# kit-cel/vae-equalizer

Hardware: AMD Instinct MI355X
Metric: equalized symbols/s/GPU, DP 64-QAM VAE-LE (higher is better)
Workload: dtype f32

## Files before the change

### vae_equalizer_amd/csrc/vaeq_dp_wave_kernel.h

```cpp
#pragma once
#include <hip/hip_runtime.h>
#include <stdint.h>
#include <type_traits>

#include "vaeq.h"
#include "vaeq_common.h"
#include "vaeq_launch.h"
#include "vaeq_wave.h"

#ifdef VAEQ_PHASE_STAMPS
#define VAEQ_STAMP(i) do { if (s == a.steps - 1) tst[i] = __builtin_readcyclecounter(); } while (0)
#define VAEQ_XSTAMP(i) do { if (s == a.steps - 1) tsx[i] = __builtin_readcyclecounter(); } while (0)
#else
#define VAEQ_STAMP(i) do { } while (0)
#define VAEQ_XSTAMP(i) do { } while (0)
#endif
#define VAEQ_NSTAMP 12
#ifndef VAEQ_PIPE
#define VAEQ_PIPE 1
#endif
#ifndef VAEQ_PIPE_DU
#define VAEQ_PIPE_DU 0
#endif
#ifndef VAEQ_ROW_STEP
#define VAEQ_ROW_STEP 1
#endif
#define VAEQ_BT_FRAMES 16
#ifndef VAEQ_DEMAP_SHIFT
#define VAEQ_DEMAP_SHIFT 0
#endif
#ifndef VAEQ_WPS
#define VAEQ_WPS 2
#endif
#ifndef VAEQ_CHAIN_BOUND
#define VAEQ_CHAIN_BOUND 0
#endif
#ifndef VAEQ_HALF_SWAP
#define VAEQ_HALF_SWAP 1
#endif
#ifndef VAEQ_QST_OFF
#define VAEQ_QST_OFF 0
#endif
#ifndef VAEQ_QST_NOWAIT
#define VAEQ_QST_NOWAIT 1
#endif
#ifndef VAEQ_QST_NT
#define VAEQ_QST_NT 1
#endif

namespace vaeq {

#if VAEQ_CHAIN_BOUND
__device__ __forceinline__ float chain_sum(float v) { asm volatile("" :: "v"(v)); return 1.0f; }
__device__ __forceinline__ float chain_scan(float v) { return v; }
__device__ __forceinline__ float chain_half_scan(float v) { return v; }
__device__ __forceinline__ float chain_rcp(float v) { asm volatile("" :: "v"(v)); return 1.0f; }
__device__ __forceinline__ float chain_log(float v) { asm volatile("" :: "v"(v)); return 1.0f; }
__device__ __forceinline__ void chain_adam(float &, float &m, float &v, float g, float, float) { m = g; v = g; }
#define VAEQ_CUT(real, cut) (cut)
#else
#define VAEQ_CUT(real, cut) (real)
__device__ __forceinline__ float chain_sum(float v) { return wave_sum_dpp(v); }
__device__ __forceinline__ float chain_scan(float v) { return wave_incl_scan_dpp(v); }
__device__ __forceinline__ float chain_half_scan(float v) { return half_incl_scan_dpp(v); }
__device__ __forceinline__ float chain_rcp(float v) { return __builtin_amdgcn_rcpf(v); }
__device__ __forceinline__ float chain_log(float v) { return __builtin_amdgcn_logf(v); }
__device__ __forceinline__ void chain_adam(float &p, float &m, float &v, float g, float ss, float bc) { adam_update_fast(p, m, v, g, ss, bc); }
#endif

template <bool DH>
__device__ __forceinline__ float half_sum(float a0, float a1, int half)
{
#if VAEQ_CHAIN_BOUND
    if constexpr (DH) return half ? a1 : a0;
#endif
    const auto r = __builtin_amdgcn_permlane32_swap(__builtin_bit_cast(unsigned, a0), __builtin_bit_cast(unsigned, a1), false, false);
    return __builtin_bit_cast(float, (unsigned)r[0]) + __builtin_bit_cast(float, (unsigned)r[1]);
}

struct WaveLayout {
    int Lph, Uph;
    int X, E, U, PSv, W, H, PSh, VS, MOM, RED, XG, total;
};

__host__ __device__ inline WaveLayout wave_layout(int B, int M, int NW = 1)
{
    WaveLayout l;
    const int len = 2 * B + M - 1;
    const int lph = wave_lph(len);
    l.Lph = lph;
    l.Uph = B / 2 + 1;
    int o = 0;
    auto take = [&](int bytes) { int r = o; o += (bytes + 15) & ~15; return r; };
    l.X = take(2 * 4 * lph * 8);
    l.E = take(2 * 4 * lph * 8);
    const int ubytes = 2 * 2 * l.Uph * 8, gbytes = 2 * B * 8;
    l.U = take(ubytes > gbytes ? ubytes : gbytes);
    l.PSv = take(2 * (B + 1) * 4);
    l.W = take(2 * M * 16);
    l.H = take(2 * 2 * (M + 1) * 8);
    l.PSh = take(2 * (M + 1) * 4);
    l.VS = take(2 * M * 4);
    l.MOM = take(16 * 64 * 4);
    l.RED = take(NW > 1 ? 64 * 4 : 0);
    l.XG = take((NW - 1) * 4 * 64 * 4);
    l.total = o;
    return l;
}

template <int M, bool INIT, bool PIPE = true, bool SPLIT = true>
__device__ __forceinline__ void pair_fir(cacc (&acc)[2][2], cacc (&accx)[2][2], const float2 *xp, int Lph, const float4 *wq)
{
    cacc (&acc2)[2][2] = SPLIT ? accx : acc;
    auto tapA = [&](int k) -> v2f { return lds2(reinterpret_cast<const float2 *>(wq + k)); };
    auto tapB = [&](int k) -> v2f { return lds2(reinterpret_cast<const float2 *>(wq + k) + 1); };
    constexpr int G = M / 4;
    auto load = [&](int g, v2f (&r)[14]) {
        const float2 *xg = xp + g;
        r[0] = lds2(xg); r[1] = lds2(xg + Lph); r[2] = lds2(xg + 2 * Lph); r[3] = lds2(xg + 3 * Lph); r[4] = lds2(xg + 1); r[5] = lds2(xg + Lph + 1);
#pragma unroll
        for (int t = 0; t < 4; t++) { r[6 + 2 * t] = tapA(4 * g + t); r[7 + 2 * t] = tapB(4 * g + t); }
    };
    auto fma = [&](int, const v2f (&r)[14], auto first) {
        constexpr bool F = decltype(first)::value;
        cmacf<F>(acc[0][0], r[6], r[0]); cmacf<F>(acc[0][1], r[7], r[0]); cmacf<F>(acc[1][0], r[6], r[2]); cmacf<F>(acc[1][1], r[7], r[2]);
        cmacf<F && SPLIT>(acc2[0][0], r[8], r[1]); cmacf<F && SPLIT>(acc2[0][1], r[9], r[1]);
        cmacf<F && SPLIT>(acc2[1][0], r[8], r[3]); cmacf<F && SPLIT>(acc2[1][1], r[9], r[3]);
        cmac(acc[0][0], r[10], r[2]); cmac(acc[0][1], r[11], r[2]); cmac(acc[1][0], r[10], r[4]); cmac(acc[1][1], r[11], r[4]);
        cmac(acc2[0][0], r[12], r[3]); cmac(acc2[0][1], r[13], r[3]); cmac(acc2[1][0], r[12], r[5]); cmac(acc2[1][1], r[13], r[5]);
    };
    pipe2<14, INIT, PIPE>(G, load, fma);
#pragma unroll
    for (int k = 4 * G; k < M; k++) {
        const v2f a = tapA(k), b = tapB(k);
        const v2f xa = lds2(xp + (k & 3) * Lph + (k >> 2)), xb = lds2(xp + ((k + 2) & 3) * Lph + ((k + 2) >> 2));
        if (k & 1) { cmac(acc2[0][0], a, xa); cmac(acc2[0][1], b, xa); cmac(acc2[1][0], a, xb); cmac(acc2[1][1], b, xb); }
        else { cmac(acc[0][0], a, xa); cmac(acc[0][1], b, xa); cmac(acc[1][0], a, xb); cmac(acc[1][1], b, xb); }
    }
}

template <int M, bool PIPE = false, bool MERGE = true>
__device__ __forceinline__ void pair_du(cacc (&acc)[2][2][2], const float2 *ep, int Lph, const float2 *ht, int MP)
{
    constexpr int G = M / 4;
    auto load1 = [&](int chi, int g, v2f *x) {
        const float2 *xg = ep + chi * 4 * Lph + g;
        x[0] = lds2(xg); x[1] = lds2(xg + Lph); x[2] = lds2(xg + 2 * Lph); x[3] = lds2(xg + 3 * Lph); x[4] = lds2(xg + 1); x[5] = lds2(xg + Lph + 1);
#pragma unroll
        for (int t = 0; t < 4; t++) { x[6 + 2 * t] = lds2(ht + (chi * 2 + 0) * MP + 4 * g + t); x[7 + 2 * t] = lds2(ht + (chi * 2 + 1) * MP + 4 * g + t); }
    };
    auto fma1 = [&](int chi, const v2f *x, int t, auto first) {
        constexpr bool F = decltype(first)::value;
        cmacf<F>(acc[chi][0][0], x[6 + 2 * t], x[t]); cmacf<F>(acc[chi][0][1], x[7 + 2 * t], x[t]);
        cmacf<F>(acc[chi][1][0], x[6 + 2 * t], x[t + 2]); cmacf<F>(acc[chi][1][1], x[7 + 2 * t], x[t + 2]);
    };
    if constexpr (MERGE) {
        auto load = [&](int g, v2f (&r)[28]) { load1(0, g, r); load1(1, g, r + 14); };
        auto fma = [&](int, const v2f (&r)[28], auto first) {
            fma1(0, r, 0, first); fma1(1, r + 14, 0, first);
#pragma unroll
            for (int t = 1; t < 4; t++) { fma1(0, r, t, std::false_type{}); fma1(1, r + 14, t, std::false_type{}); }
        };
        pipe2<28, true, PIPE>(G, load, fma);
    } else {
#pragma unroll
        for (int chi = 0; chi < 2; chi++) {
            auto load = [&](int g, v2f (&r)[14]) { load1(chi, g, r); };
            auto fma = [&](int, const v2f (&r)[14], auto first) {
                fma1(chi, r, 0, first);
#pragma unroll
                for (int t = 1; t < 4; t++) fma1(chi, r, t, std::false_type{});
            };
            pipe2<14, true, PIPE>(G, load, fma);
        }
    }
#pragma unroll
    for (int k = 4 * G; k < M; k++)
#pragma unroll
        for (int chi = 0; chi < 2; chi++) {
            const float2 *xp = ep + chi * 4 * Lph;
            const v2f a = lds2(ht + (chi * 2 + 0) * MP + k), b = lds2(ht + (chi * 2 + 1) * MP + k);
            const v2f xa = lds2(xp + (k & 3) * Lph + (k >> 2)), xb = lds2(xp + ((k + 2) & 3) * Lph + ((k + 2) >> 2));
            cmac(acc[chi][0][0], a, xa); cmac(acc[chi][0][1], b, xa); cmac(acc[chi][1][0], a, xb); cmac(acc[chi][1][1], b, xb);
        }
}

constexpr bool uniform_parts(int B, int M, int NP)
{
    const int mh = M / 2, nm = 2 * B - 2 * mh;
    for (int par = 0; par < 2; par++) {
        const int T = (nm - par + 1) >> 1, Th = ((T + 2 * NP - 1) / (2 * NP)) << 1;
        int n0 = -1;
        for (int part = 0; part < NP; part++) {
            const int ma = (part * Th) >> 1, e = part * Th + Th, mb = ((T < e ? T : e) + 1) >> 1;
            if (mb - ma <= 0 || (n0 >= 0 && mb - ma != n0)) return false;
            n0 = mb - ma;
        }
    }
    const int Bq = ((B + 2 * NP - 1) / (2 * NP)) << 1;
    int n0 = -1;
    for (int part = 0; part < NP; part++) {
        const int ma = (part * Bq) >> 1, e = part * Bq + Bq, mb = (B < e ? B : e) >> 1;
        if (mb - ma <= 0 || (n0 >= 0 && mb - ma != n0)) return false;
        n0 = mb - ma;
    }
    return true;
}

template <int M, int NLEV, int BT, bool PAIR, int OUT, int NW = 1, int BL = 0>
__global__ __launch_bounds__(64 * NW, VAEQ_WPS) void dp_wave_kernel(const vaeq_dp_args a)
{
    constexpr int mh = M / 2, Mh = 2 * mh, MP = M + 1;
    constexpr float LOG2E = 1.4426950408889634f, LN2 = 0.6931471805599453f;
    extern __shared__ float4 smem4[];
    char *sm = reinterpret_cast<char *>(smem4);
    const int gl = threadIdx.x, lane = NW > 1 ? (gl & 63) : gl, wv = NW > 1 ? (gl >> 6) : 0, run = blockIdx.x;
    constexpr int NT = 64 * NW, NP = 2 * NW;
    constexpr bool UNI = BT > 0 && uniform_parts(BT, M, NP);
    constexpr bool FIXL = BT > 0 || (BL > 0 && M != 13 && M != 17 && !(M == 31 && NW == 1));
    constexpr bool PIPE = VAEQ_PIPE && FIXL;
    constexpr bool WIDE = FIXL;
    constexpr bool SWAPH = VAEQ_HALF_SWAP && BT == 100 && NW == 1;
    constexpr bool PFLAT = VAEQ_QST_NOWAIT && BT == 100 && NW == 1;
    constexpr int QAUX = VAEQ_QST_NT && BT == 100 && NW == 1 ? 2 : 0;
    constexpr bool PIPE_DU = VAEQ_PIPE_DU;
    const int B = BT ? BT : a.B;
    const int BS = BT ? BT : BL ? BL : B;
    constexpr bool ODDB = BT == 0 && BL > 0;
    const int L = 2 * B, nm = L - Mh, P2 = ODDB ? (B + 1) / 2 : B / 2;
    const float rnm = 1.0f / (float)nm;
    const WaveLayout lay = wave_layout(BS, M, NW);
    const int Lph = lay.Lph, Uph = lay.Uph;
    float2 *Xs = reinterpret_cast<float2 *>(sm + lay.X), *Es = reinterpret_cast<float2 *>(sm + lay.E);
    float2 *Us = reinterpret_cast<float2 *>(sm + lay.U), *GY = Us;
    float4 *Wt = reinterpret_cast<float4 *>(sm + lay.W);
    float2 *Ht = reinterpret_cast<float2 *>(sm + lay.H);
    float *PSv = reinterpret_cast<float *>(sm + lay.PSv);
    float *PSh = reinterpret_cast<float *>(sm + lay.PSh);
    float *VS = reinterpret_cast<float *>(sm + lay.VS);
    float *RED = reinterpret_cast<float *>(sm + lay.RED), *XG = reinterpret_cast<float *>(sm + lay.XG);

    float amp[NLEV], b2[NLEV], nlogP[NLEV];
    const float nusc = a.nu_sc[run];
#pragma unroll
    for (int i = 0; i < NLEV; i++) {
        amp[i] = a.amp[i];
        b2[i] = nusc * amp[i] * amp[i] * LOG2E;
        nlogP[i] = -logf(a.P[(size_t)run * NLEV + i]);
    }
    const float var0 = a.var[run * 2 + 0], var1 = a.var[run * 2 + 1];
    const float lrW = a.lr_W[run], lrH = a.lr_h[run];
    const float lev_delta = amp[NLEV - 1] - amp[NLEV - 2], lev_inv = 1.0f / lev_delta, lev_off = -amp[0] * lev_inv;

    for (int i = gl; i < (lay.W - lay.X) / 8; i += NT) Xs[i] = make_float2(0.f, 0.f);
    for (int i = gl; i < (lay.PSh - lay.H) / 8; i += NT) Ht[i] = make_float2(0.f, 0.f);
    __syncthreads();
    const int tk = lane & 31, half = lane >> 5;
    const bool worker = tk < M, owner = worker && wv == 0;
    const int part = wv * 2 + half;
    const size_t gbase = (size_t)run * 8 * M;
    float *MOM = reinterpret_cast<float *>(sm + lay.MOM) + lane;
#define mWr(p) MOM[(0 + (p)) * 64]
#define mWi(p) MOM[(2 + (p)) * 64]
#define vWr(p) MOM[(4 + (p)) * 64]
#define vWi(p) MOM[(6 + (p)) * 64]
#define mHr(p) MOM[(8 + (p)) * 64]
#define mHi(p) MOM[(10 + (p)) * 64]
#define vHr(p) MOM[(12 + (p)) * 64]
#define vHi(p) MOM[(14 + (p)) * 64]
    if (owner) {
#pragma unroll
        for (int p = 0; p < 2; p++) {
            const size_t ir = gbase + (half * 4 + p) * M + tk, ii = gbase + (half * 4 + 2 + p) * M + tk;
            float *wq = reinterpret_cast<float *>(&Wt[p * M + tk]);
            wq[half * 2 + 0] = a.W[ir];
            wq[half * 2 + 1] = a.W[ii];
            mWr(p) = a.adam_mW[ir]; mWi(p) = a.adam_mW[ii];
            vWr(p) = a.adam_vW[ir]; vWi(p) = a.adam_vW[ii];
            const size_t hr = gbase + ((half * 2 + p) * 2 + 0) * M + tk, hi = hr + M;
            Ht[(half * 2 + p) * MP + tk] = make_float2(a.h[hr], a.h[hi]);
            mHr(p) = a.adam_mh[hr]; mHi(p) = a.adam_mh[hi];
            vHr(p) = a.adam_vh[hr]; vHi(p) = a.adam_vh[hi];
        }
    }
    int step = a.step[run];
    __shared__ double BTW[2][VAEQ_BT_FRAMES];
    if (gl < VAEQ_BT_FRAMES && gl < a.n_frames) {
        const double t = (double)(step + gl * a.steps);
        BTW[0][gl] = pow(0.9, t);
        BTW[1][gl] = pow(0.999, t);
    }
    __syncthreads();
    double b1t = BTW[0][0], b2t = BTW[1][0];

    const int klen = a.keep_len, k0 = a.keep_off;
    const size_t No = (size_t)a.steps * klen;
    constexpr bool pairst = PAIR;
    const bool act = gl < P2;
    const int nq = (nm + 3) / 4;
    const int n0 = 2 * gl;
    const bool v1 = ODDB ? act && (n0 + 1 < B) : act;
    const float2 *Xl = Xs + gl, *El = Es + gl, *Ul = Us + gl;
    const float2 *Xa = Xs + (act ? gl : 0), *Ea = Es + (act ? gl : 0);

    const bool ldl = gl < (ODDB ? (L + 3) / 4 : L / 4);
    float4 pf[4];
    const uint32_t S4 = (uint32_t)a.S * 4u;
    auto frame_rsrc = [&](int f) { return make_rsrc(a.rx + ((size_t)run * a.n_frames + f) * 4 * (size_t)a.S, 4u * S4); };
    auto fetch = [&](const __amdgpu_buffer_rsrc_t xr, int s) {
        const uint32_t vo = ldl ? ((uint32_t)s * (uint32_t)a.stride_sym * 2u + 4u * gl) * 4u : OOB;
#pragma unroll
        for (int r = 0; r < 4; r++) pf[r] = bld128(xr, vo, (uint32_t)r * S4);
    };
#ifdef VAEQ_PHASE_STAMPS
    long long tst[VAEQ_NSTAMP], tsx[8];
#endif
    fetch(frame_rsrc(0), 0);
    for (int f = 0; f < a.n_frames; f++) {
        const __amdgpu_buffer_rsrc_t xr = frame_rsrc(f), xn = frame_rsrc(f + 1 < a.n_frames ? f + 1 : f);
        if (f && f < VAEQ_BT_FRAMES) {
            b1t = BTW[0][f];
            b2t = BTW[1][f];
        }
        const bool qf = !VAEQ_QST_OFF && OUT != 2 && a.q_out, yf = a.y_out, ef = OUT != 1 && a.eq_out, df = OUT != 1 && a.dec_out;
        const uint32_t No4 = (uint32_t)No * 4u;
        const size_t fr = (size_t)run * a.n_frames + f;
        const __amdgpu_buffer_rsrc_t qr = make_rsrc(qf ? a.q_out + fr * (4 * NLEV) * No : nullptr, qf ? 4u * NLEV * No4 : 0u);
        const __amdgpu_buffer_rsrc_t yr = make_rsrc(yf ? a.y_out + fr * 4 * No : nullptr, yf ? 4u * No4 : 0u);
        const __amdgpu_buffer_rsrc_t er = make_rsrc(ef ? a.eq_out + fr * 2 * No : nullptr, ef ? 2u * No4 : 0u);
        const __amdgpu_buffer_rsrc_t dr = make_rsrc(df ? a.dec_out + fr * 4 * No : nullptr, df ? (uint32_t)(4 * No) : 0u);
        const __amdgpu_buffer_rsrc_t lr_ = make_rsrc(a.loss ? a.loss + fr * a.steps : nullptr, a.loss ? (uint32_t)a.steps * 4u : 0u);
        const __amdgpu_buffer_rsrc_t vr_ = make_rsrc(a.var_est ? a.var_est + fr * 2 * a.steps : nullptr, a.var_est ? (uint32_t)a.steps * 8u : 0u);
#pragma unroll 1
        for (int s = 0; s < a.steps; s++) {
            VAEQ_STAMP(0);
            if (ldl) {
#pragma unroll
                for (int p = 0; p < 2; p++) {
                    const float4 I4 = pf[p * 2 + 0], Q4 = pf[p * 2 + 1];
                    const float xi[4] = {I4.x, I4.y, I4.z, I4.w}, xq[4] = {Q4.x, Q4.y, Q4.z, Q4.w};
#pragma unroll
                    for (int i = 0; i < 4; i++) {
                        const int c = mh + i;
                        const bool in = !ODDB || 4 * gl + i < L;
                        Xs[(p * 4 + (c & 3)) * Lph + gl + (c >> 2)] = in ? make_float2(xi[i], xq[i]) : make_float2(0.f, 0.f);
                    }
                }
            }
            sync_lds<NW>();

            VAEQ_STAMP(1);
            float2 y[2][2];
            {
                cacc ya[2][2], yb[2][2];
                pair_fir<M, true, PIPE, WIDE>(ya, yb, Xa, Lph, Wt);
                pair_fir<M, false, PIPE, WIDE>(ya, yb, Xa + 4 * Lph, Lph, Wt + M);
#pragma unroll
                for (int sy = 0; sy < 2; sy++)
#pragma unroll
                    for (int o = 0; o < 2; o++) {
                        if constexpr (WIDE) {
                            ya[sy][o].a += yb[sy][o].a;
                            ya[sy][o].b += yb[sy][o].b;
                        }
                        y[sy][o] = cfin(ya[sy][o]);
                    }
            }
            asm volatile("" : "+v"(y[0][0].x), "+v"(y[0][0].y), "+v"(y[0][1].x), "+v"(y[0][1].y), "+v"(y[1][0].x), "+v"(y[1][0].y),
                         "+v"(y[1][1].x), "+v"(y[1][1].y));
            VAEQ_STAMP(2);
            const bool kept0 = act && (n0 >= k0) && (n0 < k0 + klen), kept1 = act && (n0 + 1 >= k0) && (n0 + 1 < k0 + klen);
            const uint32_t col = (uint32_t)(s * klen + (n0 - k0));
            const uint32_t vo0 = kept0 ? col * 4u : OOB, vo1 = kept1 ? col * 4u + 4u : OOB;
            if (yf) {
                uint32_t yrow = 0u;
                auto next_row = [&]() {
#if VAEQ_ROW_STEP
                    yrow += No4;
                    asm volatile("" : "+s"(yrow));
#endif
                };
#pragma unroll
                for (int o = 0; o < 2; o++) {
#if VAEQ_ROW_STEP
                    const uint32_t r0 = yrow;
                    next_row();
                    const uint32_t r1 = yrow;
                    next_row();
#else
                    const uint32_t r0 = (uint32_t)(o * 2 + 0) * No4, r1 = (uint32_t)(o * 2 + 1) * No4;
#endif
                    if (pairst) {
                        bst64(v2f{y[0][o].x, y[1][o].x}, yr, vo0, r0);
                        bst64(v2f{y[0][o].y, y[1][o].y}, yr, vo0, r1);
                    } else {
                        bst32(y[0][o].x, yr, vo0, r0); bst32(y[0][o].y, yr, vo0, r1);
                        bst32(y[1][o].x, yr, vo1, r0); bst32(y[1][o].y, yr, vo1, r1);
                    }
                }
            }

            VAEQ_STAMP(3);
            float mv[2][2][2], mt3[2][2][2], mkc[2][2][2];
#if VAEQ_ROW_STEP
            uint32_t qrow = 0u;
#endif
            float klsum = 0.f, vv[2][2];
#pragma unroll
            for (int o = 0; o < 2; o++) {
                const float c2 = 0.5f / (o ? var1 : var0) * LOG2E;
                float2 muv[2];
#pragma unroll
                for (int c = 0; c < 2; c++) {
                    const v2f yy = c ? v2f{y[0][o].y, y[1][o].y} : v2f{y[0][o].x, y[1][o].x};
                    v2f z[NLEV], q[NLEV];
                    v2f ssum = {0.f, 0.f};
#if VAEQ_DEMAP_SHIFT
                    v2f dm2;
                    {
                        const v2f t = yy * lev_inv + lev_off;
                        const v2f r = {__builtin_amdgcn_fmed3f(__builtin_rintf(t.x), 0.f, (float)(NLEV - 1)), __builtin_amdgcn_fmed3f(__builtin_rintf(t.y), 0.f, (float)(NLEV - 1))};
                        const v2f dm = (t - r) * lev_delta;
                        dm2 = dm * dm;
                    }
#pragma unroll
                    for (int i = 0; i < NLEV; i++) {
                        const v2f d = yy - amp[i];
                        z[i] = -((d * d - dm2) * c2 + b2[i]);
                        q[i] = v2f{__builtin_amdgcn_exp2f(z[i].x), __builtin_amdgcn_exp2f(z[i].y)};
                        ssum += q[i];
                    }
#else
                    float zm0 = -3.0e38f, zm1 = -3.0e38f;
#pragma unroll
                    for (int i = 0; i < NLEV; i++) {
                        const v2f d = yy - amp[i];
                        z[i] = -(d * d * c2 + b2[i]);
                        zm0 = fmaxf(zm0, z[i].x);
                        zm1 = fmaxf(zm1, z[i].y);
                    }
                    const v2f zmax = {zm0, zm1};
#pragma unroll
                    for (int i = 0; i < NLEV; i++) {
                        z[i] -= zmax;
                        q[i] = v2f{__builtin_amdgcn_exp2f(z[i].x), __builtin_amdgcn_exp2f(z[i].y)};
                        ssum += q[i];
                    }
#endif
                    const v2f rs = {__builtin_amdgcn_rcpf(ssum.x), __builtin_amdgcn_rcpf(ssum.y)};
                    v2f m1 = {0.f, 0.f};
#pragma unroll
                    for (int i = 0; i < NLEV; i++) {
                        q[i] *= rs;
                        m1 += q[i] * amp[i];
                    }
                    if (ef && c == 0) {
// ... 27 lines not shown
                    if (inr1) klsum += kl.y - __builtin_amdgcn_logf(ssum.y) * LN2;
                    asm volatile("" : "+v"(m2), "+v"(m3), "+v"(kk), "+v"(klsum));
                    mv[0][o][c] = m2.x; mv[1][o][c] = m2.y;
                    mt3[0][o][c] = m3.x; mt3[1][o][c] = m3.y;
                    mkc[0][o][c] = inr0 ? kk.x : 0.f;
                    mkc[1][o][c] = inr1 ? kk.y : 0.f;
                    if (c) { muv[0].y = m1.x; muv[1].y = m1.y; } else { muv[0].x = m1.x; muv[1].x = m1.y; }
                    if (qf) {
#pragma unroll
                        for (int i = 0; i < NLEV; i++) {
#if VAEQ_ROW_STEP
                            const uint32_t ro = qrow;
#else
                            const uint32_t ro = (uint32_t)(o * 2 * NLEV + c * NLEV + i) * No4;
#endif
                            if (pairst) bst64<QAUX>(q[i], qr, vo0, ro);
                            else { bst32<QAUX>(q[i].x, qr, vo0, ro); bst32<QAUX>(q[i].y, qr, vo1, ro); }
#if VAEQ_ROW_STEP
                            qrow += No4;
                            asm volatile("" : "+s"(qrow));
#endif
                        }
                    }
                }
                vv[o][0] = act ? mv[0][o][0] + mv[0][o][1] : 0.f;
                vv[o][1] = v1 ? mv[1][o][0] + mv[1][o][1] : 0.f;
                if (act) {
                    Us[(o * 2 + 0) * Uph + gl] = muv[0];
                    Us[(o * 2 + 1) * Uph + gl] = v1 ? muv[1] : make_float2(0.f, 0.f);
                }
            }
            VAEQ_STAMP(4);
            {
                float inc[2];
#pragma unroll
                for (int o = 0; o < 2; o++) inc[o] = chain_scan(vv[o][0] + vv[o][1]);
                if constexpr (NW > 1) {
                    if (lane == 63) { RED[wv] = inc[0]; RED[NW + wv] = inc[1]; }
                    sync_lds<NW>();
#pragma unroll
                    for (int w = 0; w < NW - 1; w++)
                        if (w < wv) { inc[0] += RED[w]; inc[1] += RED[NW + w]; }
                }
#pragma unroll
                for (int o = 0; o < 2; o++) {
                    if (act) {
                        PSv[o * (BS + 1) + n0 + 1] = inc[o] - vv[o][1];
                        PSv[o * (BS + 1) + n0 + 2] = inc[o];
                    }
                    if (gl == 0) PSv[o * (BS + 1)] = 0.f;
                }
            }
            sync_lds<NW>();
            if (owner) {
                const int lo = (Mh - tk + 1) >> 1, hi_ = (nm - 1 + Mh - tk) >> 1;
                VS[half * M + tk] = VAEQ_CUT(PSv[half * (BS + 1) + hi_ + 1] - PSv[half * (BS + 1) + lo], 1.0f);
            }
            sync_lds<NW>();

            VAEQ_STAMP(5);
            float se0 = 0.f, se1 = 0.f;
            float hq0 = 0.f, hq1 = 0.f;
            if (worker) {
                const float2 h0 = Ht[(0 * 2 + half) * MP + tk], h1 = Ht[(1 * 2 + half) * MP + tk];
                hq0 = h0.x * h0.x + h0.y * h0.y;
                hq1 = h1.x * h1.x + h1.y * h1.y;
            }
            const float vsl = worker ? VAEQ_CUT(VS[half * M + tk], 1.0f) : 0.f;
            {
                cacc D[2][4];
                constexpr int NA = mh + 1, NB = NA / 2;
#pragma unroll
                for (int v = 0; v < 2; v++) {
                    const float2 *h0 = Ht + (0 * 2 + v) * MP, *h1 = Ht + (1 * 2 + v) * MP;
                    const float2 *up = Us + (gl < nq ? gl : 0) + v * 2 * Uph;
                    auto step_a = [&](int aa, v2f ulo, v2f uhi, auto first) {
                        constexpr bool F = decltype(first)::value;
                        const v2f e0 = lds2(h0 + 2 * aa), o0 = lds2(h0 + 2 * aa + 1), e1 = lds2(h1 + 2 * aa), o1 = lds2(h1 + 2 * aa + 1);
                        cmacf<F>(D[0][0], e0, ulo); cmacf<F>(D[0][1], o0, ulo);
                        cmacf<F>(D[0][2], e0, uhi); cmacf<F>(D[0][3], o0, uhi);
                        cmacf<F>(D[1][0], e1, ulo); cmacf<F>(D[1][1], o1, ulo);
                        cmacf<F>(D[1][2], e1, uhi); cmacf<F>(D[1][3], o1, uhi);
                    };
                    if (NA & 1) {
                        if (v == 0) step_a(mh, lds2(up), lds2(up + Uph), std::true_type{});
                        else step_a(mh, lds2(up), lds2(up + Uph), std::false_type{});
                    } else if (v == 0) {
#pragma unroll
                        for (int chi = 0; chi < 2; chi++)
#pragma unroll
                            for (int i = 0; i < 4; i++) D[chi][i] = cacc0();
                    }
                    constexpr int ph = mh & 1;
                    auto load = [&](int b, v2f (&r)[11]) {
                        const int sl = (mh >> 1) - b;
                        r[0] = lds2(up + ph * Uph + sl);
                        r[1] = lds2(up + (ph ^ 1) * Uph + sl + ph);
                        r[2] = lds2(up + (ph ^ 1) * Uph + sl + ph - 1);
#pragma unroll
                        for (int t = 0; t < 4; t++) { r[3 + t] = lds2(h0 + 4 * b + t); r[7 + t] = lds2(h1 + 4 * b + t); }
                    };
                    auto fma = [&](int, const v2f (&r)[11], auto) {
                        cmac(D[0][0], r[3], r[0]); cmac(D[0][1], r[4], r[0]); cmac(D[0][2], r[3], r[1]); cmac(D[0][3], r[4], r[1]);
                        cmac(D[1][0], r[7], r[0]); cmac(D[1][1], r[8], r[0]); cmac(D[1][2], r[7], r[1]); cmac(D[1][3], r[8], r[1]);
                        cmac(D[0][0], r[5], r[2]); cmac(D[0][1], r[6], r[2]); cmac(D[0][2], r[5], r[0]); cmac(D[0][3], r[6], r[0]);
                        cmac(D[1][0], r[9], r[2]); cmac(D[1][1], r[10], r[2]); cmac(D[1][2], r[9], r[0]); cmac(D[1][3], r[10], r[0]);
                    };
                    pipe2<11, false, PIPE>(NB, load, fma);
                }
                VAEQ_STAMP(6);
                if (gl < nq) {
#pragma unroll
                    for (int chi = 0; chi < 2; chi++)
#pragma unroll
                        for (int i = 0; i < 4; i++) {
                            const int ce = Mh + i;
                            const float2 x = Xl[(chi * 4 + (ce & 3)) * Lph + (ce >> 2)];
                            const float2 Dv = cfin(D[chi][i]);
                            float2 e = make_float2(x.x - Dv.x, x.y - Dv.y);
                            if (4 * gl + i >= nm) e = make_float2(0.f, 0.f);
                            Es[(chi * 4 + (ce & 3)) * Lph + gl + (ce >> 2)] = e;
                            const float e2 = e.x * e.x + e.y * e.y;
                            if (chi) se1 += e2; else se0 += e2;
                        }
                }
            }
            se0 = chain_sum(se0);
            se1 = chain_sum(se1);
            klsum = chain_sum(klsum);
            if constexpr (NW > 1) {
                if (lane == 0) { RED[16 + wv] = se0; RED[16 + NW + wv] = se1; RED[16 + 2 * NW + wv] = klsum; }
                sync_lds<NW>();
                se0 = RED[16]; se1 = RED[16 + NW]; klsum = RED[16 + 2 * NW];
#pragma unroll
                for (int w = 1; w < NW; w++) { se0 += RED[16 + w]; se1 += RED[16 + NW + w]; klsum += RED[16 + 2 * NW + w]; }
            }
            const float C0 = se0 + chain_sum(hq0 * vsl), C1 = se1 + chain_sum(hq1 * vsl);
            const float gC0 = (float)nm * chain_rcp(C0), gC1 = (float)nm * chain_rcp(C1);
            {
                const uint32_t vo = gl == 0 ? 0u : OOB;
                if (a.loss) bst32((float)nm * LN2 * (chain_log(C0) + chain_log(C1)) + klsum, lr_, vo, (uint32_t)s * 4u);
                if (a.var_est) {
                    bst32(C0 * rnm, vr_, vo, (uint32_t)s * 4u);
                    bst32(C1 * rnm, vr_, vo, ((uint32_t)a.steps + (uint32_t)s) * 4u);
                }
            }
            {
                const float inc = chain_half_scan(gC0 * hq0 + gC1 * hq1);
                if (owner) PSh[half * MP + tk + 1] = inc;
                if (tk == 0) PSh[half * MP] = 0.f;
            }
            sync_lds<NW>();

            VAEQ_STAMP(7);
            step += 1;
            b1t *= 0.9;
            b2t *= 0.999;
            const float rbc1 = VAEQ_CUT(__builtin_amdgcn_rcpf((float)(1.0 - b1t)), 1.0f);
            const float bc2s = VAEQ_CUT(__builtin_amdgcn_rcpf(__builtin_amdgcn_sqrtf((float)(1.0 - b2t))), 1.0f);
            const float ssW = lrW * rbc1, ssH = lrH * rbc1;
            float2 hnew[2];
            hnew[0] = hnew[1] = make_float2(0.f, 0.f);
            float ghr[2] = {0, 0}, ghi[2] = {0, 0};
            float2 hacc[2];
            {
                float2 ph_h[2] = {make_float2(0.f, 0.f), make_float2(0.f, 0.f)};
                float ph_vs[2] = {0.f, 0.f};
                if (NW == 1 && owner) {
#pragma unroll
                    for (int v = 0; v < 2; v++) {
                        ph_h[v] = Ht[(half * 2 + v) * MP + tk];
                        ph_vs[v] = VAEQ_CUT(VS[v * M + tk], 1.0f);
                    }
                }
                cacc ca[2][2];
                {
                    const int tkc = worker ? tk : 0, par = tkc & 1, aa = tkc >> 1;
                    const int T = (nm - par + 1) >> 1, Th = ((T + 2 * NP - 1) / (2 * NP)) << 1;
                    const int ma = (part * Th) >> 1, mb = (min(T, part * Th + Th) + 1) >> 1;
                    const int ceA = par + Mh, ceB = par + Mh + 2, npA = mh - aa, npB = mh - aa + 1;
                    const float2 *eA = Es + (ceA & 3) * Lph + (ceA >> 2) + ma, *eB = Es + (ceB & 3) * Lph + (ceB >> 2) + ma;
                    const float2 *uA = Us + (npA & 1) * Uph + (npA >> 1) + ma, *uB = Us + (npB & 1) * Uph + (npB >> 1) + ma;
                    auto load1 = [&](int m, v2f *r) {
                        r[0] = lds2(eA + m); r[1] = lds2(eA + 4 * Lph + m); r[2] = lds2(uA + m); r[3] = lds2(uA + 2 * Uph + m);
                        r[4] = lds2(eB + m); r[5] = lds2(eB + 4 * Lph + m); r[6] = lds2(uB + m); r[7] = lds2(uB + 2 * Uph + m);
                    };
                    cacc cbx[2][2];
                    cacc (&cb)[2][2] = WIDE ? cbx : ca;
                    auto fma1 = [&](const v2f *r, auto first) {
                        constexpr bool F = decltype(first)::value;
                        cmacf<F>(ca[0][0], r[2], r[0]); cmacf<F>(ca[0][1], r[3], r[0]); cmacf<F>(ca[1][0], r[2], r[1]); cmacf<F>(ca[1][1], r[3], r[1]);
                        cmacf<F && WIDE>(cb[0][0], r[6], r[4]); cmacf<F && WIDE>(cb[0][1], r[7], r[4]); cmacf<F && WIDE>(cb[1][0], r[6], r[5]); cmacf<F && WIDE>(cb[1][1], r[7], r[5]);
                    };
                    auto load = [&](int i, v2f (&r)[16]) { load1(2 * i, r); load1(2 * i + 1, r + 8); };
                    auto fma = [&](int, const v2f (&r)[16], auto first) { fma1(r, first); fma1(r + 8, std::false_type{}); };
                    int n = mb - ma;
                    VAEQ_XSTAMP(0);
                    if constexpr (UNI) {
                        n = __builtin_amdgcn_readfirstlane(n);
                        pipe2<16, true, PIPE>(n >> 1, load, fma);
                    } else {
                        ca[0][0] = ca[0][1] = ca[1][0] = ca[1][1] = cbx[0][0] = cbx[0][1] = cbx[1][0] = cbx[1][1] = cacc0();
                        pipe2<16, false, PIPE>(n >> 1, load, fma);
                    }
                    if (n & 1) {
                        v2f r[8];
                        load1(n - 1, r);
                        fma1(r, std::false_type{});
                    }
                    if constexpr (WIDE) {
#pragma unroll
                        for (int i = 0; i < 2; i++)
#pragma unroll
                            for (int j = 0; j < 2; j++) { ca[i][j].a += cbx[i][j].a; ca[i][j].b += cbx[i][j].b; }
                    }
                }
                VAEQ_XSTAMP(1);
                float2 acc[2][2];
#pragma unroll
                for (int chi = 0; chi < 2; chi++)
#pragma unroll
                    for (int v = 0; v < 2; v++) acc[chi][v] = cfinc(ca[chi][v]);
// ... 163 lines not shown
                        pipe2<16, false, PIPE>(n >> 1, load, fma);
                    }
                    if (n & 1) {
                        v2f r[8];
                        load1(n - 1, r);
                        fma1(r, std::false_type{});
                    }
                    if constexpr (WIDE) {
#pragma unroll
                        for (int i = 0; i < 2; i++)
#pragma unroll
                            for (int j = 0; j < 2; j++) { ca[i][j].a += cbx[i][j].a; ca[i][j].b += cbx[i][j].b; }
                    }
                }
                VAEQ_XSTAMP(5);
                float2 acc[2][2];
#pragma unroll
                for (int o = 0; o < 2; o++)
#pragma unroll
                    for (int pp = 0; pp < 2; pp++) acc[o][pp] = cfinc(ca[o][pp]);
                if constexpr (SWAPH) {
#pragma unroll
                    for (int p = 0; p < 2; p++) {
                        acc[0][p].x = acc[1][p].x = half_sum<false>(acc[0][p].x, acc[1][p].x, half);
                        acc[0][p].y = acc[1][p].y = half_sum<false>(acc[0][p].y, acc[1][p].y, half);
                    }
                } else {
#pragma unroll
                    for (int o = 0; o < 2; o++)
#pragma unroll
                        for (int p = 0; p < 2; p++) {
                            acc[o][p].x += __shfl_xor(acc[o][p].x, 32, 64);
                            acc[o][p].y += __shfl_xor(acc[o][p].y, 32, 64);
                        }
                }
                if constexpr (NW > 1) {
#pragma unroll
                    for (int p = 0; p < 2; p++) {
                        const float2 ac = half ? acc[1][p] : acc[0][p];
                        if (wv > 0) {
                            XG[((wv - 1) * 4 + 2 * p + 0) * 64 + lane] = ac.x;
                            XG[((wv - 1) * 4 + 2 * p + 1) * 64 + lane] = ac.y;
                        }
                    }
                    sync_lds<NW>();
                }
                VAEQ_XSTAMP(6);
                if (owner) {
#pragma unroll
                    for (int p = 0; p < 2; p++) {
                        float2 ac = half ? acc[1][p] : acc[0][p];
                        if constexpr (NW > 1) {
#pragma unroll
                            for (int w = 0; w < NW - 1; w++) {
                                ac.x += XG[(w * 4 + 2 * p + 0) * 64 + lane];
                                ac.y += XG[(w * 4 + 2 * p + 1) * 64 + lane];
                            }
                        }
                        gwr[p] = ac.x;
                        gwi[p] = ac.y;
                        if (!a.no_update) {
                            float *wq = reinterpret_cast<float *>(&Wt[p * M + tk]) + half * 2;
                            float wr = pw_w[p][0], wi = pw_w[p][1];
                            chain_adam(wr, pw_m[p][0], pw_v[p][0], gwr[p], ssW, bc2s);
                            chain_adam(wi, pw_m[p][1], pw_v[p][1], gwi[p], ssW, bc2s);
                            wq[0] = wr;
                            wq[1] = wi;
                            mWr(p) = pw_m[p][0]; mWi(p) = pw_m[p][1];
                            vWr(p) = pw_v[p][0]; vWi(p) = pw_v[p][1];
                        }
                    }
                }
            }
            if (a.dbg_gW && owner && f == a.n_frames - 1 && s == a.steps - 1) {
#pragma unroll
                for (int p = 0; p < 2; p++) {
                    a.dbg_gW[gbase + (half * 4 + p) * M + tk] = gwr[p];
                    a.dbg_gW[gbase + (half * 4 + 2 + p) * M + tk] = gwi[p];
                    a.dbg_gh[gbase + ((half * 2 + p) * 2 + 0) * M + tk] = ghr[p];
                    a.dbg_gh[gbase + ((half * 2 + p) * 2 + 1) * M + tk] = ghi[p];
                }
            }
            sync_lds<NW>();
            VAEQ_XSTAMP(7);
            VAEQ_STAMP(11);
        }
    }
#ifdef VAEQ_PHASE_STAMPS
    if (gl == 0 && run == (int)gridDim.x / 2 && a.loss)
        for (int i = 0; i + 1 < VAEQ_NSTAMP; i++) a.loss[i] = (float)(tst[i + 1] - tst[i]);
    if (gl == 0 && run == (int)gridDim.x / 2 && a.loss)
        for (int i = 0; i < 7; i++) a.loss[16 + i] = (float)(tsx[i + 1] - tsx[i]);
#endif

    if (owner && !a.no_update) {
#pragma unroll
        for (int p = 0; p < 2; p++) {
            const size_t ir = gbase + (half * 4 + p) * M + tk, ii = gbase + (half * 4 + 2 + p) * M + tk;
            const float *wq = reinterpret_cast<const float *>(&Wt[p * M + tk]) + half * 2;
            a.W[ir] = wq[0]; a.W[ii] = wq[1];
            a.adam_mW[ir] = mWr(p); a.adam_mW[ii] = mWi(p);
            a.adam_vW[ir] = vWr(p); a.adam_vW[ii] = vWi(p);
            const size_t hr = gbase + ((half * 2 + p) * 2 + 0) * M + tk, hi = hr + M;
            const float2 hh = Ht[(half * 2 + p) * MP + tk];
            a.h[hr] = hh.x; a.h[hi] = hh.y;
            a.adam_mh[hr] = mHr(p); a.adam_mh[hi] = mHi(p);
            a.adam_vh[hr] = vHr(p); a.adam_vh[hi] = vHi(p);
        }
    }
    if (gl == 0 && !a.no_update) a.step[run] = step;
#undef mWr
#undef mWi
#undef vWr
#undef vWi
#undef mHr
#undef mHi
#undef vHr
#undef vHi
}


template <int M, int NLEV, int BT, int NW>
static int launch_wave(const vaeq_dp_args &a, hipStream_t st)
{
    const size_t lds = (size_t)wave_layout(a.B, M, NW).total;
    const bool pair = ((a.keep_len | a.keep_off) & 1) == 0;
    void (*k)(const vaeq_dp_args) = pair ? dp_wave_kernel<M, NLEV, BT, true, 0, NW> : dp_wave_kernel<M, NLEV, BT, false, 0, NW>;
    if (BT) {
        if (!a.eq_out && !a.dec_out) k = pair ? dp_wave_kernel<M, NLEV, BT, true, BT ? 1 : 0, NW> : dp_wave_kernel<M, NLEV, BT, false, BT ? 1 : 0, NW>;
        else if (!a.q_out) k = pair ? dp_wave_kernel<M, NLEV, BT, true, BT ? 2 : 0, NW> : dp_wave_kernel<M, NLEV, BT, false, BT ? 2 : 0, NW>;
    }
    const int out = !BT ? 0 : (!a.eq_out && !a.dec_out) ? 1 : !a.q_out ? 2 : 0;
    note_kernel("vaeq::dp_wave_kernel<%d, %d, %d, %s, %d, %d, 0>", M, NLEV, BT, pair ? "true" : "false", out, NW);
    return launch(k, dim3(a.R), dim3(64 * NW), lds, st, a);
}

template <int M, int NLEV, int BL, int NW, bool SPEC = true>
static int launch_wave_fixl(const vaeq_dp_args &a, hipStream_t st)
{
    const size_t lds = (size_t)wave_layout(BL, M, NW).total;
    const bool pair = ((a.keep_len | a.keep_off) & 1) == 0;
    const int out = !SPEC ? 0 : (!a.eq_out && !a.dec_out) ? 1 : !a.q_out ? 2 : 0;
    void (*k)(const vaeq_dp_args) = pair ? dp_wave_kernel<M, NLEV, 0, true, 0, NW, BL> : dp_wave_kernel<M, NLEV, 0, false, 0, NW, BL>;
    if constexpr (SPEC) {
        if (out == 1) k = pair ? dp_wave_kernel<M, NLEV, 0, true, 1, NW, BL> : dp_wave_kernel<M, NLEV, 0, false, 1, NW, BL>;
        else if (out == 2) k = pair ? dp_wave_kernel<M, NLEV, 0, true, 2, NW, BL> : dp_wave_kernel<M, NLEV, 0, false, 2, NW, BL>;
    }
    note_kernel("vaeq::dp_wave_kernel<%d, %d, 0, %s, %d, %d, %d>", M, NLEV, pair ? "true" : "false", out, NW, BL);
    return launch(k, dim3(a.R), dim3(64 * NW), lds, st, a);
}

template <int M, int NLEV, int BL, int NW>
static int64_t wave_resident_fixl()
{
    int nb = 0, dev = 0;
    hipDeviceProp_t prop;
    if (hipGetDevice(&dev) != hipSuccess || hipGetDeviceProperties(&prop, dev) != hipSuccess) return VAEQ_ERR_DEVICE;
    auto k = dp_wave_kernel<M, NLEV, 0, true, 0, NW, BL>;
    if (hipOccupancyMaxActiveBlocksPerMultiprocessor(&nb, k, 64 * NW, (size_t)wave_layout(BL, M, NW).total) != hipSuccess) return VAEQ_ERR_DEVICE;
    return (int64_t)nb * prop.multiProcessorCount;
}

template <int M, int BT, int NW>
static int launch_wave_lev(const vaeq_dp_args &a, hipStream_t st)
{
    return dispatch_nlev(a.n_lev, [&](auto nl) { return launch_wave<M, decltype(nl)::value, BT, NW>(a, st); });
// ... 61 lines not shown
```

### vae_equalizer_amd/csrc/vaeq_wave.h

```cpp
#pragma once
#include <hip/hip_runtime.h>
#include <stdint.h>
#include <type_traits>

#ifndef VAEQ_SUM_BCAST
#define VAEQ_SUM_BCAST 1
#endif

namespace vaeq {

__device__ __forceinline__ void wave_lds_sync() { asm volatile("" ::: "memory"); }

template <int NW>
__device__ __forceinline__ void sync_lds()
{
    if constexpr (NW == 1) wave_lds_sync();
    else asm volatile("s_waitcnt lgkmcnt(0)\n\ts_barrier" ::: "memory");
}

template <int NW, int K>
__device__ __forceinline__ void waves_sum(float (&v)[K], float *red, int lane, int wv)
{
    if constexpr (NW > 1) {
        if (lane == 0) {
// ... 100 lines not shown
    v2f A[NR], B[NR];
    load(0, A);
    load(1, B);
    fma(0, A, std::integral_constant<bool, INIT>{});
    int i = 1;
#pragma unroll 1
    for (; i + 1 < n; i += 2) {
        load(i + 1, A);
        fma(i, B, std::false_type{});
        load(i + 2, B);
        fma(i + 1, A, std::false_type{});
    }
    if (i < n) fma(i, B, std::false_type{});
}

__device__ __forceinline__ v2f cfin2(const cacc &c)
{
    v2f r;
    asm("v_pk_add_f32 %0, %1, %2 op_sel:[0,1] op_sel_hi:[1,0] neg_lo:[0,1]" : "=v"(r) : "v"(c.a), "v"(c.b));
    return r;
}
__device__ __forceinline__ v2f cfinc2(const cacc &c)
{
    v2f r;
    asm("v_pk_add_f32 %0, %1, %2 op_sel:[0,1] op_sel_hi:[1,0] neg_hi:[0,1]" : "=v"(r) : "v"(c.a), "v"(c.b));
    return r;
}
__device__ __forceinline__ float2 cfin(const cacc &c) { const v2f r = cfin2(c); return make_float2(r.x, r.y); }
__device__ __forceinline__ float2 cfinc(const cacc &c) { const v2f r = cfinc2(c); return make_float2(r.x, r.y); }

template <int CTRL, int ROW_MASK = 0xF, int BANK_MASK = 0xF>
__device__ __forceinline__ float dpp_f(float v)
{
    return __builtin_bit_cast(float, __builtin_amdgcn_update_dpp(0, __builtin_bit_cast(int, v), CTRL, ROW_MASK, BANK_MASK, true));
}
__device__ __forceinline__ float wave_sum_dpp(float v)
{
    v += dpp_f<0xB1>(v);
    v += dpp_f<0x4E>(v);
    v += dpp_f<0x141>(v);
    v += dpp_f<0x140>(v);
#if VAEQ_SUM_BCAST
    v += dpp_f<0x142, 0xA>(v);
    v += dpp_f<0x143, 0xC>(v);
    return __builtin_bit_cast(float, __builtin_amdgcn_readlane(__builtin_bit_cast(int, v), 63));
#endif
    const int b = __builtin_bit_cast(int, v);
    const float r0 = __builtin_bit_cast(float, __builtin_amdgcn_readlane(b, 0)), r1 = __builtin_bit_cast(float, __builtin_amdgcn_readlane(b, 16));
    const float r2 = __builtin_bit_cast(float, __builtin_amdgcn_readlane(b, 32)), r3 = __builtin_bit_cast(float, __builtin_amdgcn_readlane(b, 48));
    return (r0 + r1) + (r2 + r3);
}
__device__ __forceinline__ float row_incl_scan_dpp(float v)
{
    float s = v + dpp_f<0x111>(v);
    s += dpp_f<0x112>(v);
    s += dpp_f<0x113>(v);
    s += dpp_f<0x114, 0xF, 0xE>(s);
    s += dpp_f<0x118, 0xF, 0xC>(s);
    return s;
}
__device__ __forceinline__ float half_incl_scan_dpp(float v)
{
    float s = row_incl_scan_dpp(v);
    s += dpp_f<0x142, 0xA>(s);
    return s;
}
__device__ __forceinline__ float wave_incl_scan_dpp(float v)
{
    float s = half_incl_scan_dpp(v);
    s += dpp_f<0x143, 0xC>(s);
    return s;
}

__device__ __forceinline__ float wave_incl_scan(float v, int lane)
{
#pragma unroll
    for (int d = 1; d < 64; d <<= 1) {
        const float t = __shfl_up(v, d, 64);
        if (lane >= d) v += t;
    }
    return v;
}

__host__ __device__ inline int wave_lph(int len)
{
    int lph = (len + 3) / 4 + 1;
    while ((lph & 31) != 8 && (lph & 31) != 24) lph++;
    return lph;
}

}
```

Measured before the change: 10.68 billion.

## Batch per-step loss and variance stores through LDS; drop padded tap and column math

Per-step loss and variance estimates are staged in an LDS ring of 100 rows and flushed to global memory in bulk with coalesced buffer stores, replacing single-lane scalar stores every step. The D-gradient accumulation skips the odd padded tap when mh is even and initialises the accumulators in the first pipelined pass. Store column offsets are carried incrementally across steps instead of recomputed. This costs extra LDS, guarded by a static assert that eight waves still fit per CU, and adds a periodic flush with a wave sync.

```diff
diff --git a/vae_equalizer_amd/csrc/vaeq_dp_wave_kernel.h b/vae_equalizer_amd/csrc/vaeq_dp_wave_kernel.h
--- a/vae_equalizer_amd/csrc/vaeq_dp_wave_kernel.h
+++ b/vae_equalizer_amd/csrc/vaeq_dp_wave_kernel.h
@@ -46,6 +46,17 @@
 #endif
 #ifndef VAEQ_QST_NT
 #define VAEQ_QST_NT 1
+#endif
+
+#ifndef VAEQ_LOSS_LDS
+#define VAEQ_LOSS_LDS 1
+#endif
+#define VAEQ_LOSS_ROWS 100
+#ifndef VAEQ_D_NOPAD
+#define VAEQ_D_NOPAD 1
+#endif
+#ifndef VAEQ_COL_STEP
+#define VAEQ_COL_STEP 1
 #endif
 
 namespace vaeq {
@@ -80,12 +91,12 @@
 
 struct WaveLayout {
     int Lph, Uph;
-    int X, E, U, PSv, W, H, PSh, VS, MOM, RED, XG, total;
+    int X, E, U, PSv, W, H, PSh, VS, MOM, RED, XG, LV, total;
 };
 
-__host__ __device__ inline WaveLayout wave_layout(int B, int M, int NW = 1)
-{
-    WaveLayout l;
+__host__ __device__ constexpr WaveLayout wave_layout_c(int B, int M, int NW)
+{
+    WaveLayout l{};
     const int len = 2 * B + M - 1;
     const int lph = wave_lph(len);
     l.Lph = lph;
@@ -104,9 +115,12 @@
     l.MOM = take(16 * 64 * 4);
     l.RED = take(NW > 1 ? 64 * 4 : 0);
     l.XG = take((NW - 1) * 4 * 64 * 4);
+    l.LV = take(VAEQ_LOSS_LDS && B == 100 && NW == 1 ? 3 * VAEQ_LOSS_ROWS * 4 : 0);
     l.total = o;
     return l;
 }
+__host__ __device__ inline WaveLayout wave_layout(int B, int M, int NW = 1) { return wave_layout_c(B, M, NW); }
+static_assert(8 * wave_layout_c(100, 25, 1).total <= 160 * 1024, "B = 100 layout: 8 resident waves per CU no longer fit the LDS");
 
 template <int M, bool INIT, bool PIPE = true, bool SPLIT = true>
 __device__ __forceinline__ void pair_fir(cacc (&acc)[2][2], cacc (&accx)[2][2], const float2 *xp, int Lph, const float4 *wq)
@@ -223,6 +237,9 @@
     constexpr bool SWAPH = VAEQ_HALF_SWAP && BT == 100 && NW == 1;
     constexpr bool PFLAT = VAEQ_QST_NOWAIT && BT == 100 && NW == 1;
     constexpr int QAUX = VAEQ_QST_NT && BT == 100 && NW == 1 ? 2 : 0;
+    constexpr bool LVLDS = VAEQ_LOSS_LDS && BT == 100 && NW == 1;
+    constexpr bool NOPAD = VAEQ_D_NOPAD && BT == 100 && NW == 1 && !(mh & 1);
+    constexpr bool COLSTEP = VAEQ_COL_STEP && BT == 100 && NW == 1;
     constexpr bool PIPE_DU = VAEQ_PIPE_DU;
     const int B = BT ? BT : a.B;
     const int BS = BT ? BT : BL ? BL : B;
@@ -239,6 +256,7 @@
     float *PSh = reinterpret_cast<float *>(sm + lay.PSh);
     float *VS = reinterpret_cast<float *>(sm + lay.VS);
     float *RED = reinterpret_cast<float *>(sm + lay.RED), *XG = reinterpret_cast<float *>(sm + lay.XG);
+    float *LV = reinterpret_cast<float *>(sm + lay.LV);
 
     float amp[NLEV], b2[NLEV], nlogP[NLEV];
     const float nusc = a.nu_sc[run];
@@ -331,6 +349,12 @@
         const __amdgpu_buffer_rsrc_t dr = make_rsrc(df ? a.dec_out + fr * 4 * No : nullptr, df ? (uint32_t)(4 * No) : 0u);
         const __amdgpu_buffer_rsrc_t lr_ = make_rsrc(a.loss ? a.loss + fr * a.steps : nullptr, a.loss ? (uint32_t)a.steps * 4u : 0u);
         const __amdgpu_buffer_rsrc_t vr_ = make_rsrc(a.var_est ? a.var_est + fr * 2 * a.steps : nullptr, a.var_est ? (uint32_t)a.steps * 8u : 0u);
+        int lrow = 0;
+        uint32_t vo0r = OOB, vo1r = OOB;
+        if constexpr (COLSTEP) {
+            if (act && (n0 >= k0) && (n0 < k0 + klen)) vo0r = (uint32_t)(n0 - k0) * 4u;
+            if (act && (n0 + 1 >= k0) && (n0 + 1 < k0 + klen)) vo1r = (uint32_t)(n0 + 1 - k0) * 4u;
+        }
 #pragma unroll 1
         for (int s = 0; s < a.steps; s++) {
             VAEQ_STAMP(0);
@@ -371,7 +395,8 @@
             VAEQ_STAMP(2);
             const bool kept0 = act && (n0 >= k0) && (n0 < k0 + klen), kept1 = act && (n0 + 1 >= k0) && (n0 + 1 < k0 + klen);
             const uint32_t col = (uint32_t)(s * klen + (n0 - k0));
-            const uint32_t vo0 = kept0 ? col * 4u : OOB, vo1 = kept1 ? col * 4u + 4u : OOB;
+            const uint32_t vo0 = COLSTEP ? vo0r : kept0 ? col * 4u : OOB, vo1 = COLSTEP ? vo1r : kept1 ? col * 4u + 4u : OOB;
+            if constexpr (COLSTEP) { vo0r += (uint32_t)klen * 4u; vo1r += (uint32_t)klen * 4u; }
             if (yf) {
                 uint32_t yrow = 0u;
                 auto next_row = [&]() {
@@ -565,7 +590,16 @@
                         cmacf<F>(D[1][0], e1, ulo); cmacf<F>(D[1][1], o1, ulo);
                         cmacf<F>(D[1][2], e1, uhi); cmacf<F>(D[1][3], o1, uhi);
                     };
-                    if (NA & 1) {
+                    auto step_e = [&](v2f ulo, v2f uhi, auto first) {
+                        constexpr bool F = decltype(first)::value;
+                        const v2f e0 = lds2(h0 + 2 * mh), e1 = lds2(h1 + 2 * mh);
+                        cmacf<F>(D[0][0], e0, ulo); cmacf<F>(D[0][2], e0, uhi);
+                        cmacf<F>(D[1][0], e1, ulo); cmacf<F>(D[1][2], e1, uhi);
+                    };
+                    if constexpr (NOPAD) {
+                        if (v == 0) step_e(lds2(up), lds2(up + Uph), std::true_type{});
+                        else step_e(lds2(up), lds2(up + Uph), std::false_type{});
+                    } else if (NA & 1) {
                         if (v == 0) step_a(mh, lds2(up), lds2(up + Uph), std::true_type{});
                         else step_a(mh, lds2(up), lds2(up + Uph), std::false_type{});
                     } else if (v == 0) {
@@ -583,13 +617,17 @@
 #pragma unroll
                         for (int t = 0; t < 4; t++) { r[3 + t] = lds2(h0 + 4 * b + t); r[7 + t] = lds2(h1 + 4 * b + t); }
                     };
-                    auto fma = [&](int, const v2f (&r)[11], auto) {
-                        cmac(D[0][0], r[3], r[0]); cmac(D[0][1], r[4], r[0]); cmac(D[0][2], r[3], r[1]); cmac(D[0][3], r[4], r[1]);
-                        cmac(D[1][0], r[7], r[0]); cmac(D[1][1], r[8], r[0]); cmac(D[1][2], r[7], r[1]); cmac(D[1][3], r[8], r[1]);
+                    auto fma = [&](int, const v2f (&r)[11], auto first) {
+                        constexpr bool F = NOPAD && decltype(first)::value;
+                        cmac(D[0][0], r[3], r[0]); cmacf<F>(D[0][1], r[4], r[0]); cmac(D[0][2], r[3], r[1]); cmacf<F>(D[0][3], r[4], r[1]);
+                        cmac(D[1][0], r[7], r[0]); cmacf<F>(D[1][1], r[8], r[0]); cmac(D[1][2], r[7], r[1]); cmacf<F>(D[1][3], r[8], r[1]);
                         cmac(D[0][0], r[5], r[2]); cmac(D[0][1], r[6], r[2]); cmac(D[0][2], r[5], r[0]); cmac(D[0][3], r[6], r[0]);
                         cmac(D[1][0], r[9], r[2]); cmac(D[1][1], r[10], r[2]); cmac(D[1][2], r[9], r[0]); cmac(D[1][3], r[10], r[0]);
                     };
-                    pipe2<11, false, PIPE>(NB, load, fma);
+                    if constexpr (NOPAD) {
+                        if (v == 0) pipe2<11, true, PIPE>(NB, load, fma);
+                        else pipe2<11, false, PIPE>(NB, load, fma);
+                    } else pipe2<11, false, PIPE>(NB, load, fma);
                 }
                 VAEQ_STAMP(6);
                 if (gl < nq) {
@@ -620,7 +658,14 @@
             }
             const float C0 = se0 + chain_sum(hq0 * vsl), C1 = se1 + chain_sum(hq1 * vsl);
             const float gC0 = (float)nm * chain_rcp(C0), gC1 = (float)nm * chain_rcp(C1);
-            {
+            if constexpr (LVLDS) {
+                if (gl == 0) {
+                    LV[lrow] = (float)nm * LN2 * (chain_log(C0) + chain_log(C1)) + klsum;
+                    LV[VAEQ_LOSS_ROWS + lrow] = C0 * rnm;
+                    LV[2 * VAEQ_LOSS_ROWS + lrow] = C1 * rnm;
+                }
+                lrow++;
+            } else {
                 const uint32_t vo = gl == 0 ? 0u : OOB;
                 if (a.loss) bst32((float)nm * LN2 * (chain_log(C0) + chain_log(C1)) + klsum, lr_, vo, (uint32_t)s * 4u);
                 if (a.var_est) {
@@ -950,6 +995,25 @@
                 }
             }
             sync_lds<NW>();
+            if constexpr (LVLDS) {
+                if (lrow == VAEQ_LOSS_ROWS || s + 1 == a.steps) {
+                    const size_t s0 = (size_t)(s + 1 - lrow);
+                    const uint32_t nb = (uint32_t)lrow * 4u;
+                    const __amdgpu_buffer_rsrc_t lf = make_rsrc(a.loss ? a.loss + fr * a.steps + s0 : nullptr, a.loss ? nb : 0u);
+                    const __amdgpu_buffer_rsrc_t v0f = make_rsrc(a.var_est ? a.var_est + fr * 2 * a.steps + s0 : nullptr, a.var_est ? nb : 0u);
+                    const __amdgpu_buffer_rsrc_t v1f = make_rsrc(a.var_est ? a.var_est + (fr * 2 + 1) * a.steps + s0 : nullptr, a.var_est ? nb : 0u);
+#pragma unroll
+                    for (int i0 = 0; i0 < VAEQ_LOSS_ROWS; i0 += 64) {
+                        const int i = i0 + gl, ic = min(i, VAEQ_LOSS_ROWS - 1);
+                        const uint32_t vo = i < lrow ? (uint32_t)i * 4u : OOB;
+                        bst32(LV[ic], lf, vo, 0u);
+                        bst32(LV[VAEQ_LOSS_ROWS + ic], v0f, vo, 0u);
+                        bst32(LV[2 * VAEQ_LOSS_ROWS + ic], v1f, vo, 0u);
+                    }
+                    lrow = 0;
+                    wave_lds_sync();
+                }
+            }
             VAEQ_XSTAMP(7);
             VAEQ_STAMP(11);
         }
diff --git a/vae_equalizer_amd/csrc/vaeq_wave.h b/vae_equalizer_amd/csrc/vaeq_wave.h
--- a/vae_equalizer_amd/csrc/vaeq_wave.h
+++ b/vae_equalizer_amd/csrc/vaeq_wave.h
@@ -206,7 +206,7 @@
     return v;
 }
 
-__host__ __device__ inline int wave_lph(int len)
+__host__ __device__ constexpr int wave_lph(int len)
 {
     int lph = (len + 3) / 4 + 1;
     while ((lph & 31) != 8 && (lph & 31) != 24) lph++;
```

Result: no change. 10.72 billion, median of 6 (+0.4%).
